# google-ai-edge/ai-edge-quantizer

Measured on AMD Instinct MI355X. Metric: weight-bytes quantized/sec (GB/s), 4096x4096 per-channel int8, higher is better.
Workload: dtype f32; 1 GPU; per-channel int8 symmetric requant of 4096x4096 FP32 weight buffers (BASELINE config 2)

## Files before the change

### ai-edge-quantizer_amd/csrc/reduce_exact.hip

```cpp
#include <cstdlib>

#include "common.h"

namespace mi355q {
namespace {

constexpr int kChunk = 8192;

__device__ __forceinline__ float lane_bcast(float v, int src_lane) {
  return __int_as_float(__builtin_amdgcn_readlane(__float_as_int(v), src_lane));
}

__device__ __forceinline__ float wave_shr1(float v) {
  return __int_as_float(__builtin_amdgcn_update_dpp(0, __float_as_int(v), 0x138, 0xF, 0xF, false));
}

template <bool SQUARE>
__device__ __forceinline__ float tr(float v) {
  if constexpr (SQUARE) return v * v;
  return v;
}

template <bool SQUARE>
__device__ __forceinline__ float leaf_sum(const float* a, int m, int lane) {
  const int full = m & ~7;
  float r = 0.f;
  if (lane < 8) {
    r = tr<SQUARE>(a[lane]);
    for (int i = 8; i < full; i += 8) r = r + tr<SQUARE>(a[i + lane]);
  }
  const float r0 = lane_bcast(r, 0), r1 = lane_bcast(r, 1), r2 = lane_bcast(r, 2),
              r3 = lane_bcast(r, 3), r4 = lane_bcast(r, 4), r5 = lane_bcast(r, 5),
              r6 = lane_bcast(r, 6), r7 = lane_bcast(r, 7);
  float res = ((r0 + r1) + (r2 + r3)) + ((r4 + r5) + (r6 + r7));
  for (int i = full; i < m; ++i) res = res + tr<SQUARE>(a[i]);
  return res;
}

template <bool SQUARE, int DEPTH>
__device__ __noinline__ float pairwise_sum(const float* a, int n, int lane) {
  if (n < 8) {
    float res = 0.f;
    for (int i = 0; i < n; ++i) res = res + tr<SQUARE>(a[i]);
    return res;
  }
  if (n <= 128) return leaf_sum<SQUARE>(a, n, lane);
  if constexpr (DEPTH > 0) {
    int n2 = n / 2;
    n2 -= n2 % 8;
    const float left = pairwise_sum<SQUARE, DEPTH - 1>(a, n2, lane);
    const float right = pairwise_sum<SQUARE, DEPTH - 1>(a + n2, n - n2, lane);
    return left + right;
  } else {
    return leaf_sum<SQUARE>(a, n, lane);
  }
}

struct RunSum {
  float acc = 0.f;
  unsigned count = 0;
  int pend_start = 0;
  int pend_len = 0;
  float pend_sum = 0.f;

  __device__ __forceinline__ void flush(const float* a, int lane) {
    if (pend_len > 0) {
      acc = acc + (pend_len < 8 ? pend_sum : pairwise_sum<false, 8>(a + pend_start, pend_len, lane));
      pend_len = 0;
    }
  }

  __device__ __forceinline__ void feed(unsigned long long m, int base, float v, const float* a,
                                       int lane) {
    if ((base % kChunk) == 0 || (m & 1ull) == 0) flush(a, lane);
    count += static_cast<unsigned>(__builtin_popcountll(m));
    if (m == 0) return;
    const unsigned long long m4 = m & (m >> 1) & (m >> 2) & (m >> 3);
    if ((m4 & (m4 >> 4)) != 0 || (pend_len > 0 && pend_len + __builtin_ctzll(~m) >= 8)) {
      feed_runs(m, base, v, a, lane);
      return;
    }
    const float carry = pend_len > 0 ? pend_sum : 0.f;
    pend_len = 0;
    const bool sel = ((m >> lane) & 1ull) != 0;
    float partial = sel ? (lane == 0 ? carry : 0.f) + v : 0.f;
    const unsigned long long m2 = m & (m >> 1);
    if (m2 != 0) {
      const bool cont = (((m2 << 1) >> lane) & 1ull) != 0;
      const int rounds = (m2 & (m >> 2)) == 0 ? 1 : (m4 == 0 ? 2 : 6);
      for (int t = 0; t < rounds; ++t) {
        const float left = wave_shr1(partial);
        if (cont) partial = left + v;
      }
    }
    unsigned long long mf = m;
    if (m >> 63) {
      const int t = __builtin_clzll(~m);
      mf = m & (~0ull >> t);
      pend_start = base + 64 - t;
      pend_len = t;
      pend_sum = lane_bcast(partial, 63);
    }
    unsigned long long ends = mf & ~(mf >> 1);
    const int k = __builtin_popcountll(ends);
    if (k <= 3) {
      while (ends != 0) {
        acc = acc + lane_bcast(partial, __builtin_ctzll(ends));
        ends &= ends - 1ull;
      }
      return;
    }
    const bool is_end = ((ends >> lane) & 1ull) != 0;
    const int rank = __builtin_amdgcn_mbcnt_hi(static_cast<unsigned>(ends >> 32),
                                               __builtin_amdgcn_mbcnt_lo(static_cast<unsigned>(ends), 0));
    const int dest = is_end ? rank : k + lane - rank;
    const float r = __int_as_float(__builtin_amdgcn_ds_permute(dest << 2, __float_as_int(partial)));
    float x = r;
    for (int t = 0; t < k; t += 4) {
#pragma unroll
      for (int j = 0; j < 4; ++j) {
        const float left = __int_as_float(__builtin_amdgcn_update_dpp(
            __float_as_int(acc), __float_as_int(x), 0x138, 0xF, 0xF, false));
        x = left + r;
      }
    }
    acc = lane_bcast(x, k - 1);
  }

  __device__ __forceinline__ float chain(float start, float v, int s, int len) {
    float rs = start;
    for (int i = 0; i < len; ++i) rs = rs + lane_bcast(v, s + i);
    return rs;
  }

  __device__ __forceinline__ void feed_runs(unsigned long long m, int base, float v, const float* a,
                                            int lane) {
    while (m != 0) {
      const int s = __builtin_ctzll(m);
      const unsigned long long t = m >> s;
      const int len = (~t == 0) ? 64 - s : __builtin_ctzll(~t);
      if (s + len == 64) {
        if (pend_len > 0) {
          pend_len += len;
        } else {
          pend_start = base + s;
          pend_len = len;
          if (len < 8) pend_sum = chain(0.f, v, s, len);
        }
        return;
      }
      if (pend_len > 0) {
        if (pend_len + len < 8) {
          acc = acc + chain(pend_sum, v, 0, len);
          pend_len = 0;
        } else {
          pend_len += len;
          flush(a, lane);
        }
      } else if (len < 8) {
        acc = acc + chain(0.f, v, s, len);
      } else {
        acc = acc + pairwise_sum<false, 8>(a + base + s, len, lane);
      }
      m &= ~(((1ull << len) - 1ull) << s);
    }
  }
};

template <bool USE_LDS>
__device__ __forceinline__ const float* stage_unit(const float* g, int len, float* lds, int lane) {
  if constexpr (!USE_LDS) return g;
  if ((reinterpret_cast<uintptr_t>(g) & 15) == 0) {
    const int n4 = len / 4;
    const float4* g4 = reinterpret_cast<const float4*>(g);
    float4* l4 = reinterpret_cast<float4*>(lds);
    for (int i = lane; i < n4; i += kWave) l4[i] = g4[i];
    for (int i = n4 * 4 + lane; i < len; i += kWave) lds[i] = g[i];
  } else {
    for (int i = lane; i < len; i += kWave) lds[i] = g[i];
  }
  return lds;
}

struct OctavArgs {
  const float* x;
  long long units;
  int len;
  int lds_stride;
  int max_iter;
  int count_is_f64;
  float s;
  float* hist;
  unsigned long long* moving;
  struct TailState* tail;
  float* tail_values;
  unsigned short* tail_pos;
  int tail_cap;
};

struct TailState {
  int next_it;
  int n[2];
  float guess;
  float cand_guess;
  unsigned moved_lo, moved_hi;
  int pad;
};

struct OctavStep {
  float next;
  bool close;
};

__device__ __forceinline__ OctavStep octav_step(float guess, float pos_sum, float neg_sum,
                                                long long pos_count, long long neg_count,
                                                long long len, float s, int count_is_f64) {
  const float num = pos_sum - neg_sum;
  float den = static_cast<float>(pos_count);
  den = static_cast<float>(static_cast<double>(den) + static_cast<double>(neg_count));
  den = den * (1.0f - s);
  if (count_is_f64)
    den = static_cast<float>(static_cast<double>(den) +
                             static_cast<double>(s) * static_cast<double>(len));
  else
    den = den + s * static_cast<float>(len);
  const float next = num / den;
  const float tol = 1e-8f + 1e-5f * fabsf(next);
  const bool close = (fabsf(guess - next) <= tol && __builtin_isfinite(next)) || guess == next;
  return {next, close};
}

__device__ __forceinline__ void publish_moving(unsigned long long* flags, unsigned long long moved) {
  if (moved == 0) return;
  const unsigned long long seen = __atomic_load_n(flags, __ATOMIC_RELAXED);
  if ((seen & moved) != moved) atomicOr(flags, moved);
}

__device__ __forceinline__ bool reached_fixed_point(float guess, float next) { return next == guess; }

__device__ __forceinline__ void repeat_iterate(const OctavArgs& a, int it, long long unit, float value) {
  for (int r = it + 1; r < a.max_iter; ++r) a.hist[static_cast<long long>(r) * a.units + unit] = value;
}

template <bool USE_LDS>
__global__ void octav_kernel(OctavArgs a) {
  extern __shared__ __attribute__((aligned(16))) float smem[];
  const int lane = threadIdx.x & (kWave - 1);
  const int wave = threadIdx.x / kWave;
  const long long unit = static_cast<long long>(blockIdx.x) * (blockDim.x / kWave) + wave;
  const bool live = unit < a.units;
  const float* u = nullptr;
  if (live)
    u = stage_unit<USE_LDS>(a.x + unit * a.len, a.len, smem + static_cast<size_t>(wave) * a.lds_stride, lane);
  if constexpr (USE_LDS) __syncthreads();
  if (!live) return;

  const int len = a.len;
  const float qnan = __builtin_nanf("");
  float guess = 1.0f;
  unsigned long long moved = 0;
  for (int it = 0; it < a.max_iter; ++it) {
    RunSum pos, neg;
    const float hi = guess, lo = -guess;
    for (int base = 0; base < len; base += kWave) {
      const int i = base + lane;
      const float v = i < len ? u[i] : qnan;
      const unsigned long long mp = __ballot(v >= hi), mn = __ballot(v <= lo);
      if ((mp | mn) == 0 && (pos.pend_len | neg.pend_len) == 0) continue;
      pos.feed(mp, base, v, u, lane);
      neg.feed(mn, base, v, u, lane);
    }
    pos.flush(u, lane);
    neg.flush(u, lane);
    const OctavStep st = octav_step(guess, pos.acc, neg.acc, pos.count, neg.count, len, a.s,
                                    a.count_is_f64);
    if (lane == 0) a.hist[static_cast<long long>(it) * a.units + unit] = st.next;
    if (!st.close) moved |= 1ull << it;
    if (reached_fixed_point(guess, st.next)) {
      if (lane == 0) repeat_iterate(a, it, unit, st.next);
      break;
    }
    guess = st.next;
  }
  if (lane == 0) publish_moving(a.moving, moved);
}

#ifndef MI355Q_ROWS_MIN_LEN
#define MI355Q_ROWS_MIN_LEN 129
#endif
constexpr int kRowsMinLen = MI355Q_ROWS_MIN_LEN, kRowsMaxLen = 2 * kChunk;
constexpr int kPiece = 16;

__device__ __forceinline__ int pidx(int e) { return e + (e >> 4); }


template <int CTRL, int ROW_MASK>
__device__ __forceinline__ int dpp_add(int x) {
  return x + __builtin_amdgcn_update_dpp(0, x, CTRL, ROW_MASK, 0xF, true);
}

__device__ __forceinline__ int wave_incl_scan(int x) {
  x = dpp_add<0x111, 0xF>(x);
  x = dpp_add<0x112, 0xF>(x);
  x = dpp_add<0x114, 0xF>(x);
  x = dpp_add<0x118, 0xF>(x);
// ... 1214 lines not shown
}

size_t octav_rows_smem(int len) {
  const int kRowsThreads = octav_rows_threads(len);
  const int npieces = (len + kPiece - 1) / kPiece;
  const size_t row_floats = static_cast<size_t>((len + (len >> 4) + 4) & ~3);
  const size_t cap = static_cast<size_t>(((len / 2 + 2 + 63) & ~63) + 64);
  return 2 * rows_xchg_floats(kRowsThreads) * sizeof(float) + kRowsThreads * sizeof(float) + row_floats * sizeof(float) + cap * 2 * sizeof(float) +
         static_cast<size_t>((npieces + 1) & ~1) * 2 * sizeof(unsigned short);
}

__global__ void octav_seg_kernel(OctavArgs a, long long channels, long long outer) {
  const int lane = threadIdx.x & (kWave - 1);
  const int wave = threadIdx.x / kWave;
  const long long c = static_cast<long long>(blockIdx.x) * (blockDim.x / kWave) + wave;
  if (c >= channels) return;
  const int inner = a.len;
  const float qnan = __builtin_nanf("");
  float guess = 1.0f;
  unsigned long long moved = 0;
  for (int it = 0; it < a.max_iter; ++it) {
    RunSum pos, neg;
    long long npos = 0, nneg = 0;
    const float hi = guess, lo = -guess;
    for (long long o = 0; o < outer; ++o) {
      const float* u = a.x + (o * channels + c) * inner;
      for (int base = 0; base < inner; base += kWave) {
        const int i = base + lane;
        const float v = i < inner ? u[i] : qnan;
        pos.feed(__ballot(v >= hi), base, v, u, lane);
        neg.feed(__ballot(v <= lo), base, v, u, lane);
      }
      pos.flush(u, lane);
      neg.flush(u, lane);
      npos += pos.count;
      nneg += neg.count;
      pos.count = neg.count = 0;
    }
    const OctavStep st = octav_step(guess, pos.acc, neg.acc, npos, nneg, outer * inner, a.s, 1);
    if (lane == 0) a.hist[static_cast<long long>(it) * a.units + c] = st.next;
    if (!st.close) moved |= 1ull << it;
    if (reached_fixed_point(guess, st.next)) {
      if (lane == 0) repeat_iterate(a, it, c, st.next);
      break;
    }
    guess = st.next;
  }
  if (lane == 0) publish_moving(a.moving, moved);
}

__global__ void mse_scale_seg_kernel(const float* __restrict__ x, long long outer, long long channels,
                                     int inner, float multiplier, float* __restrict__ scale) {
  const int lane = threadIdx.x & (kWave - 1);
  const int wave = threadIdx.x / kWave;
  const long long c = static_cast<long long>(blockIdx.x) * (blockDim.x / kWave) + wave;
  if (c >= channels) return;
  float acc = 0.f;
  bool first = true;
  for (long long o = 0; o < outer; ++o) {
    const float* u = x + (o * channels + c) * inner;
    for (int k = 0; k < inner; k += kChunk) {
      const int n = inner - k < kChunk ? inner - k : kChunk;
      const float part = pairwise_sum<true, 8>(u + k, n, lane);
      acc = first ? part : acc + part;
      first = false;
    }
  }
  const float mean = acc / static_cast<float>(outer * inner);
  if (lane == 0) scale[c] = multiplier * __builtin_sqrtf(mean);
}

constexpr int kColsUnroll = 8;

__global__ __launch_bounds__(256) void octav_cols_kernel(OctavArgs a, long long channels) {
  const long long c_raw = static_cast<long long>(blockIdx.x) * 256 + threadIdx.x;
  const bool live = c_raw < channels;
  const long long c = live ? c_raw : channels - 1;
  const long long outer = a.len;
  float guess = 1.0f;
  bool settled = false;
  unsigned long long moved = 0;
  for (int it = 0; it < a.max_iter; ++it) {
    const float hi = guess, lo = -guess;
    float pos = 0.f, neg = 0.f;
    long long npos = 0, nneg = 0;
    const float* p = a.x + c;
    long long o = 0;
    for (; o + kColsUnroll <= outer; o += kColsUnroll) {
      float v[kColsUnroll];
#pragma unroll
      for (int k = 0; k < kColsUnroll; ++k) v[k] = p[static_cast<long long>(k) * channels];
#pragma unroll
      for (int k = 0; k < kColsUnroll; ++k) {
        if (v[k] >= hi) { pos = pos + v[k]; ++npos; }
        if (v[k] <= lo) { neg = neg + v[k]; ++nneg; }
      }
      p += kColsUnroll * channels;
    }
    for (; o < outer; ++o, p += channels) {
      const float v = *p;
      if (v >= hi) { pos = pos + v; ++npos; }
      if (v <= lo) { neg = neg + v; ++nneg; }
    }
    const OctavStep st = octav_step(guess, pos, neg, npos, nneg, outer, a.s, a.count_is_f64);
    if (live && !settled) a.hist[static_cast<long long>(it) * a.units + c] = st.next;
    if (live && !settled && !st.close) moved |= 1ull << it;
    if (!settled && reached_fixed_point(guess, st.next)) {
      settled = true;
      if (live) repeat_iterate(a, it, c, st.next);
    }
    guess = st.next;
    if (__all(settled)) break;
  }
  for (int off = kWave / 2; off > 0; off >>= 1) moved |= __shfl_xor(moved, off, kWave);
  if ((threadIdx.x & (kWave - 1)) == 0) publish_moving(a.moving, moved);
}

__global__ __launch_bounds__(256) void mse_scale_cols_kernel(const float* __restrict__ x, long long outer,
                                                            long long channels, float multiplier,
                                                            float* __restrict__ scale) {
  const long long c = static_cast<long long>(blockIdx.x) * 256 + threadIdx.x;
  if (c >= channels) return;
  const float* p = x + c;
  float acc = 0.f;
  long long o = 0;
  for (; o + kColsUnroll <= outer; o += kColsUnroll) {
    float v[kColsUnroll];
#pragma unroll
    for (int k = 0; k < kColsUnroll; ++k) v[k] = p[static_cast<long long>(k) * channels];
#pragma unroll
    for (int k = 0; k < kColsUnroll; ++k) acc = acc + v[k] * v[k];
    p += kColsUnroll * channels;
  }
  for (; o < outer; ++o, p += channels) acc = acc + (*p) * (*p);
  scale[c] = multiplier * __builtin_sqrtf(acc / static_cast<float>(outer));
}

__global__ __launch_bounds__(256) void octav_pick_kernel(const float* __restrict__ hist,
                                                        const unsigned long long* __restrict__ moving,
                                                        long long units, int max_iter, int early_stop,
                                                        float* __restrict__ clip, int* iters_out) {
  int k = max_iter - 1;
  if (early_stop)
    for (int it = 0; it < max_iter; ++it)
      if (((*moving >> it) & 1ull) == 0) { k = it; break; }
  const long long i = static_cast<long long>(blockIdx.x) * 256 + threadIdx.x;
  if (i < units) clip[i] = hist[static_cast<long long>(k) * units + i];
  if (i == 0 && iters_out != nullptr) *iters_out = k + 1;
}

struct MseArgs {
  const float* x;
  long long units;
  int len;
  int lds_stride;
  float multiplier;
  float* scale;
  unsigned* q = nullptr;
  float lo = 0.f, hi = 0.f;
};

__device__ void list_leaves(int lo, int n, int* leaf_lo, int* leaf_n, int* count) {
  if (n <= 128) {
    leaf_lo[*count] = lo;
    leaf_n[*count] = n;
    ++*count;
    return;
  }
  int n2 = n / 2;
  n2 -= n2 % 8;
  list_leaves(lo, n2, leaf_lo, leaf_n, count);
  list_leaves(lo + n2, n - n2, leaf_lo, leaf_n, count);
}

__device__ float fold_leaves(int n, const float* leaf_sum, int* next) {
  if (n <= 128) return leaf_sum[(*next)++];
  int n2 = n / 2;
  n2 -= n2 % 8;
  const float left = fold_leaves(n2, leaf_sum, next);
  return left + fold_leaves(n - n2, leaf_sum, next);
}

__global__ __launch_bounds__(256) void mse_scale_leaves_kernel(MseArgs a) {
  __shared__ int leaf_lo[2][128], leaf_n[2][128], leaves[2];
  __shared__ float leaf_sum[4][128];
  const int lane = threadIdx.x & (kWave - 1), wave = threadIdx.x / kWave;
  const int k = lane & 7, slot = lane >> 3;
  const int last_len = a.len - (a.len - 1) / kChunk * kChunk;
  if (threadIdx.x == 0 || threadIdx.x == kWave) {
    const int t = threadIdx.x == 0 ? 0 : 1;
    int c = 0;
    list_leaves(0, t == 0 ? (a.len < kChunk ? a.len : kChunk) : last_len, leaf_lo[t], leaf_n[t], &c);
    leaves[t] = c;
  }
  __syncthreads();
  const long long unit = static_cast<long long>(blockIdx.x) * 4 + wave;
  const bool live_unit = unit < a.units;
  const float* u = a.x + (live_unit ? unit : 0) * a.len;
  float acc = 0.f;
  for (int c0 = 0; c0 < a.len; c0 += kChunk) {
    const int n = a.len - c0 < kChunk ? a.len - c0 : kChunk;
    const int t = (c0 + kChunk >= a.len) ? 1 : 0;
    const int count = leaves[t];
    for (int base = 0; base < count; base += 8) {
      const int leaf = base + slot;
      const bool live = leaf < count;
      const float* p = u + c0 + (live ? leaf_lo[t][leaf] : 0);
      const int ln = live ? leaf_n[t][leaf] : 0;
      float res = 0.f;
      if (ln < 8) {
        for (int i = 0; i < ln; ++i) res = res + p[i] * p[i];
      } else {
        float v[16];
#pragma unroll
        for (int q = 0; q < 16; ++q) v[q] = (8 * (q + 1) <= ln) ? p[8 * q + k] : 0.f;
        float r = v[0] * v[0];
#pragma unroll
        for (int q = 1; q < 16; ++q)
          if (8 * (q + 1) <= ln) r = r + v[q] * v[q];
        r = r + __shfl_xor(r, 1, kWave);
        r = r + __shfl_xor(r, 2, kWave);
        r = r + __shfl_xor(r, 4, kWave);
        for (int i = ln & ~7; i < ln; ++i) r = r + p[i] * p[i];
        res = r;
      }
      if (live && k == 0) leaf_sum[wave][leaf] = res;
    }
    __syncthreads();
    if (lane == 0) {
      int next = 0;
      const float part = fold_leaves(n, leaf_sum[wave], &next);
      acc = c0 == 0 ? part : acc + part;
    }
    __syncthreads();
  }
  if (lane == 0 && live_unit) {
    const float mean = acc / static_cast<float>(a.len);
    a.scale[unit] = a.multiplier * __builtin_sqrtf(mean);
  }
}

__global__ __launch_bounds__(256) void mse_scale_balanced_kernel(MseArgs a, int last_leaf, int last_depth) {
  const int lane = threadIdx.x & (kWave - 1), wave = threadIdx.x / kWave;
  const int k = lane & 7, slot = lane >> 3;
  const long long unit = static_cast<long long>(blockIdx.x) * 4 + wave;
  if (unit >= a.units) return;
  const float* u = a.x + unit * a.len;
  float acc = 0.f;
  for (int c0 = 0; c0 < a.len; c0 += kChunk) {
    const bool last = c0 + kChunk >= a.len;
    const int leaf_len = last ? last_leaf : 128, depth = last ? last_depth : 6;
    const int count = 1 << depth;
    const int steps = count > 8 ? count >> 3 : 1;
    float lvl0 = 0.f, lvl1 = 0.f, lvl2 = 0.f, x = 0.f;
#pragma unroll
    for (int s = 0; s < 8; ++s) {
      if (s < steps) {
        const int leaf = s * 8 + slot;
        const float* p = u + c0 + static_cast<long long>(leaf < count ? leaf : 0) * leaf_len + k;
        float v[16];
#pragma unroll
        for (int q = 0; q < 16; ++q) v[q] = (8 * (q + 1) <= leaf_len) ? p[8 * q] : 0.f;
        float r = v[0] * v[0];
#pragma unroll
        for (int q = 1; q < 16; ++q)
          if (8 * (q + 1) <= leaf_len) r = r + v[q] * v[q];
        r = r + __shfl_xor(r, 1, kWave);
        r = r + __shfl_xor(r, 2, kWave);
        r = r + __shfl_xor(r, 4, kWave);
        if (count > 1) r = r + __shfl_xor(r, 8, kWave);
        if (count > 2) r = r + __shfl_xor(r, 16, kWave);
        if (count > 4) r = r + __shfl_xor(r, 32, kWave);
        x = r;
        if (s & 1) {
          x = lvl0 + x;
          if (s & 2) {
            x = lvl1 + x;
            if (s & 4) x = lvl2 + x; else lvl2 = x;
          } else {
            lvl1 = x;
          }
        } else {
          lvl0 = x;
        }
      }
    }
    acc = c0 == 0 ? x : acc + x;
  }
  acc = lane_bcast(acc, 0);
  const float mean = acc / static_cast<float>(a.len);
  const float scale = a.multiplier * __builtin_sqrtf(mean);
  if (lane == 0) a.scale[unit] = scale;
  if (a.q != nullptr) {
    const float4* u4 = reinterpret_cast<const float4*>(u);
    unsigned* q = a.q + unit * (a.len / 4);
    for (int i = lane; i < a.len / 4; i += kWave) {
      const float4 v = u4[i];
      const unsigned w = (static_cast<unsigned>(round_clip(v.x / scale, a.lo, a.hi)) & 0xFFu) |
                         ((static_cast<unsigned>(round_clip(v.y / scale, a.lo, a.hi)) & 0xFFu) << 8) |
                         ((static_cast<unsigned>(round_clip(v.z / scale, a.lo, a.hi)) & 0xFFu) << 16) |
                         ((static_cast<unsigned>(round_clip(v.w / scale, a.lo, a.hi)) & 0xFFu) << 24);
      __builtin_nontemporal_store(w, q + i);
    }
  }
}

struct UnitPlan {
  bool use_lds;
  int waves;
  int lds_stride;
  size_t smem;
};

UnitPlan plan_units(int len) {
  UnitPlan p{};
  const int stride = (len + 3) / 4 * 4;
  const size_t per_wave = static_cast<size_t>(stride) * sizeof(float);
  constexpr size_t kBudget = 64 * 1024;
  int waves = static_cast<int>(kBudget / (per_wave ? per_wave : 1));
  if (waves > 4) waves = 4;
  if (waves >= 1) {
    p.use_lds = true;
    p.waves = waves;
    p.lds_stride = stride;
    p.smem = per_wave * waves;
  } else {
    p.use_lds = false;
    p.waves = 4;
    p.lds_stride = 0;
    p.smem = 0;
  }
  return p;
}


struct OctavFastArgs {
  const float* x;
  long long units;
  int len;
  int max_iter;
  float s;
  float* hist;
  unsigned long long* moving;
};

template <int CTRL>
__device__ __forceinline__ float dpp_f32(float v) {
  return __builtin_bit_cast(float, __builtin_amdgcn_update_dpp(0, __builtin_bit_cast(int, v), CTRL, 0xF, 0xF, true));
}
template <int CTRL>
__device__ __forceinline__ int dpp_i32(int v) { return __builtin_amdgcn_update_dpp(0, v, CTRL, 0xF, 0xF, true); }

template <int LANES>
__device__ __forceinline__ float unit_sum_f32(float v) {
  if constexpr (LANES >= 2) v += dpp_f32<0xB1>(v);
  if constexpr (LANES >= 4) v += dpp_f32<0x4E>(v);
  if constexpr (LANES >= 8) v += dpp_f32<0x141>(v);
  if constexpr (LANES >= 16) v += dpp_f32<0x140>(v);
  if constexpr (LANES >= 32) {
    const int b = __builtin_bit_cast(int, v);
    const float r0 = __builtin_bit_cast(float, __builtin_amdgcn_readlane(b, 0)), r1 = __builtin_bit_cast(float, __builtin_amdgcn_readlane(b, 16));
    const float r2 = __builtin_bit_cast(float, __builtin_amdgcn_readlane(b, 32)), r3 = __builtin_bit_cast(float, __builtin_amdgcn_readlane(b, 48));
    if constexpr (LANES >= 64) v = (r0 + r1) + (r2 + r3);
    else v = (threadIdx.x & 32) ? r2 + r3 : r0 + r1;
  }
  return v;
}
template <int LANES>
__device__ __forceinline__ int unit_sum_i32(int v) {
  if constexpr (LANES >= 2) v += dpp_i32<0xB1>(v);
  if constexpr (LANES >= 4) v += dpp_i32<0x4E>(v);
  if constexpr (LANES >= 8) v += dpp_i32<0x141>(v);
  if constexpr (LANES >= 16) v += dpp_i32<0x140>(v);
  if constexpr (LANES >= 32) {
    const int r0 = __builtin_amdgcn_readlane(v, 0), r1 = __builtin_amdgcn_readlane(v, 16);
    const int r2 = __builtin_amdgcn_readlane(v, 32), r3 = __builtin_amdgcn_readlane(v, 48);
    if constexpr (LANES >= 64) v = (r0 + r1) + (r2 + r3);
    else v = (threadIdx.x & 32) ? r2 + r3 : r0 + r1;
  }
  return v;
}

template <int LANES, int V>
__global__ __launch_bounds__(LANES > 256 ? LANES : 256) void octav_fast_kernel(OctavFastArgs a) {
  constexpr int THREADS = LANES > 256 ? LANES : 256;
  constexpr int UPB = THREADS / LANES;
  constexpr int WAVES = LANES / kWave;
  const int l = threadIdx.x % LANES;
  const long long u = static_cast<long long>(blockIdx.x) * UPB + threadIdx.x / LANES;
  const bool live = u < a.units;
  const int len4 = a.len / 4;
  const float4* __restrict__ x4 = reinterpret_cast<const float4*>(a.x) + (live ? u : 0) * len4;
  const float qnan = __builtin_nanf("");
  typedef float v4f __attribute__((ext_vector_type(4)));
  v4f raw[V];
#pragma unroll
  for (int j = 0; j < V; ++j) {
    const int c = j * LANES + l;
    raw[j] = __builtin_nontemporal_load(reinterpret_cast<const v4f*>(&x4[c < len4 ? c : len4 - 1]));
  }
  float v[V][4];
  int zeros = 0;
  float top = 0.f;
#pragma unroll
  for (int j = 0; j < V; ++j) {
    const bool mine = live && j * LANES + l < len4;
#pragma unroll
    for (int e = 0; e < 4; ++e) {
      v[j][e] = mine ? fabsf(raw[j][e]) : qnan;
      top = fmaxf(top, v[j][e]);
      if constexpr (LANES >= kWave) zeros += __builtin_popcountll(__builtin_amdgcn_ballot_w64(v[j][e] == 0.f));
      else zeros += v[j][e] == 0.f;
    }
  }
  __shared__ double red_sum[2][WAVES > 0 ? WAVES : 1];
  __shared__ int red_cnt[2][WAVES > 0 ? WAVES : 1];
  float unit_top = 0.f;
  if constexpr (LANES >= kWave) {
    unit_top = top;
#pragma unroll
    for (int off = kWave / 2; off > 0; off >>= 1) unit_top = fmaxf(unit_top, __shfl_xor(unit_top, off, kWave));
    if constexpr (WAVES > 1) {
      __shared__ float red_top[WAVES > 0 ? WAVES : 1];
      if ((threadIdx.x & (kWave - 1)) == 0) red_top[threadIdx.x / kWave] = unit_top;
      __syncthreads();
#pragma unroll
      for (int k = 0; k < WAVES; ++k) unit_top = fmaxf(unit_top, red_top[k]);
    }
  }
  float guess = 1.0f;
  unsigned long long moved = 0;
  int it = 0;
  for (; it < a.max_iter; ++it) {
    float part = 0.f;
    int cnt = 0;
    if constexpr (LANES >= kWave) {
      if (!(guess > unit_top)) {
        float p0 = 0.f, p1 = 0.f, p2 = 0.f, p3 = 0.f;
#pragma unroll
        for (int j = 0; j < V; ++j) {
          float t0, t1, t2, t3;
          int n0, n1, n2, n3;
          unsigned long long m0, m1, m2, m3;
          asm volatile(
              "v_cmp_ge_f32_e64 %[m0], %[x0], %[g]\n\tv_cmp_ge_f32_e64 %[m1], %[x1], %[g]\n\t"
              "v_cmp_ge_f32_e64 %[m2], %[x2], %[g]\n\tv_cmp_ge_f32_e64 %[m3], %[x3], %[g]\n\t"
              "v_cndmask_b32_e64 %[t0], 0, %[x0], %[m0]\n\tv_cndmask_b32_e64 %[t1], 0, %[x1], %[m1]\n\t"
              "v_cndmask_b32_e64 %[t2], 0, %[x2], %[m2]\n\tv_cndmask_b32_e64 %[t3], 0, %[x3], %[m3]\n\t"
              "s_bcnt1_i32_b64 %[n0], %[m0]\n\ts_bcnt1_i32_b64 %[n1], %[m1]\n\t"
              "s_bcnt1_i32_b64 %[n2], %[m2]\n\ts_bcnt1_i32_b64 %[n3], %[m3]\n\t"
              "v_add_f32 %[p0], %[p0], %[t0]\n\tv_add_f32 %[p1], %[p1], %[t1]\n\t"
              "v_add_f32 %[p2], %[p2], %[t2]\n\tv_add_f32 %[p3], %[p3], %[t3]\n\t"
              "s_add_i32 %[n0], %[n0], %[n1]\n\ts_add_i32 %[n2], %[n2], %[n3]\n\t"
              "s_add_i32 %[c], %[c], %[n0]\n\ts_add_i32 %[c], %[c], %[n2]"
              : [p0] "+v"(p0), [p1] "+v"(p1), [p2] "+v"(p2), [p3] "+v"(p3), [c] "+s"(cnt),
                [t0] "=&v"(t0), [t1] "=&v"(t1), [t2] "=&v"(t2), [t3] "=&v"(t3),
                [n0] "=&s"(n0), [n1] "=&s"(n1), [n2] "=&s"(n2), [n3] "=&s"(n3),
                [m0] "=&s"(m0), [m1] "=&s"(m1), [m2] "=&s"(m2), [m3] "=&s"(m3)
              : [x0] "v"(v[j][0]), [x1] "v"(v[j][1]), [x2] "v"(v[j][2]), [x3] "v"(v[j][3]), [g] "v"(guess)
              : "scc");
        }
        part = (p0 + p1) + (p2 + p3);
        if (guess == 0.f) cnt += zeros;
      }
    } else {
#pragma unroll
      for (int j = 0; j < V; ++j)
#pragma unroll
        for (int e = 0; e < 4; ++e) {
          const bool sel = v[j][e] >= guess;
          part += sel ? v[j][e] : 0.f;
          cnt += sel;
        }
      cnt = unit_sum_i32<LANES>(cnt + (guess == 0.f ? zeros : 0));
    }
    double sum = static_cast<double>(unit_sum_f32<(LANES < kWave ? LANES : kWave)>(part));
    if constexpr (WAVES > 1) {
      const int w = threadIdx.x / kWave, b = it & 1;
      if ((threadIdx.x & (kWave - 1)) == 0) { red_sum[b][w] = sum; red_cnt[b][w] = cnt; }
      __syncthreads();
      sum = 0.0; cnt = 0;
#pragma unroll
      for (int k = 0; k < WAVES; ++k) { sum += red_sum[b][k]; cnt += red_cnt[b][k]; }
    }
    const OctavStep st = octav_step(guess, static_cast<float>(sum), 0.f, cnt, 0, a.len, a.s, 1);
    if (live && l == 0) a.hist[static_cast<long long>(it) * a.units + u] = st.next;
    if (!st.close) moved |= 1ull << it;
    const bool fixed = reached_fixed_point(guess, st.next);
    guess = st.next;
    if constexpr (LANES >= kWave) {
      if (fixed) { ++it; break; }
    }
  }
  if constexpr (LANES >= kWave) {
    if (live && l == 0)
      for (int k = it; k < a.max_iter; ++k) a.hist[static_cast<long long>(k) * a.units + u] = guess;
  }
  if (!live) moved = 0;
#pragma unroll
  for (int off = kWave / 2; off > 0; off >>= 1) {
    const unsigned lo = __shfl_xor(static_cast<unsigned>(moved), off, kWave);
    const unsigned hi = __shfl_xor(static_cast<unsigned>(moved >> 32), off, kWave);
    moved |= (static_cast<unsigned long long>(hi) << 32) | lo;
  }
  if ((threadIdx.x & (kWave - 1)) == 0) publish_moving(a.moving, moved);
}

template <int LANES, int V>
void launch_octav_fast(const OctavFastArgs& a, hipStream_t st) {
  constexpr int THREADS = LANES > 256 ? LANES : 256;
  constexpr int UPB = THREADS / LANES;
  hipLaunchKernelGGL((octav_fast_kernel<LANES, V>), dim3(static_cast<unsigned>((a.units + UPB - 1) / UPB)), dim3(THREADS), 0, st, a);
}

}
}

using namespace mi355q;

extern "C" size_t mi355q_octav_workspace_bytes(int64_t units, int32_t max_iter) {
  if (units <= 0 || max_iter <= 0) return 0;
  return static_cast<size_t>(units) * max_iter * sizeof(float) + 64 * sizeof(int);
}

extern "C" size_t mi355q_octav_rows_workspace_bytes(int64_t units, int64_t unit_len, int32_t max_iter) {
  const size_t base = mi355q_octav_workspace_bytes(units, max_iter);
  if (base == 0 || unit_len < kRowsMinLen || unit_len > kRowsMaxLen) return base;
  const size_t cap = static_cast<size_t>(octav_tail_cap(static_cast<int>(unit_len)));
  return ((base + 63) & ~static_cast<size_t>(63)) + static_cast<size_t>(units) * (sizeof(TailState) + 2 * cap * (sizeof(float) + sizeof(unsigned short)));
}

extern "C" int32_t mi355q_octav_clip_f32(const float* x, int64_t units, int64_t unit_len,
                                         int32_t bits, int32_t max_iter, float exponent_divisor,
                                         int32_t early_stop, int32_t count_is_f64, float* clip_out,
                                         int32_t* iters_out, void* workspace,
                                         size_t workspace_bytes, void* stream) {
  clear_error();
  if (units < 0 || unit_len < 0) return fail(MI355Q_BAD_ARG, "negative shape");
  if (max_iter < 1 || max_iter > 64) return fail(MI355Q_BAD_ARG, "max_iter must be in [1, 64]");
  if (bits < 1 || bits > 16) return fail(MI355Q_BAD_ARG, "bits must be in [1, 16]");
  if (units == 0) return MI355Q_OK;
  if (unit_len == 0) return fail(MI355Q_BAD_SHAPE, "empty reduction unit");
  if (unit_len > 0x7FFFFFFFLL - 64) return fail(MI355Q_UNSUPPORTED, "unit_len too large");
  if (!x || !clip_out) return fail(MI355Q_BAD_ARG, "null pointer");
  const size_t need = mi355q_octav_workspace_bytes(units, max_iter);
  if (!workspace || workspace_bytes < need)
    return fail(MI355Q_BAD_ARG, "workspace too small: need %zu bytes", need);
  hipStream_t st = as_stream(stream);
  float* hist = static_cast<float*>(workspace);
  unsigned long long* not_close = reinterpret_cast<unsigned long long*>(hist + (units * max_iter + 1) / 2 * 2);
  if (hipMemsetAsync(not_close, 0, sizeof(unsigned long long), st) != hipSuccess)
    return fail(MI355Q_HIP_ERROR, "hipMemsetAsync failed");
  double p4 = 1.0;
  for (int i = 0; i < bits; ++i) p4 *= 0.25;
  const float s = static_cast<float>(p4 / static_cast<double>(exponent_divisor));
  if ((unit_len == 32 || unit_len == 64 || unit_len == 128 || unit_len == 256) && (reinterpret_cast<uintptr_t>(x) & 15) == 0 &&
      (units + kWave - 1) / kWave <= 0x7FFFFFFFLL && octav_unit_lanes_on() && !getenv("MI355Q_OCTAV_WAVE_KERNEL")) {
    OctavArgs a{x, units, static_cast<int>(unit_len), 0, max_iter, count_is_f64, s, hist, not_close};
    const dim3 grid(static_cast<unsigned>((units + kWave - 1) / kWave));
    if (unit_len == 32) hipLaunchKernelGGL(octav_unit_lanes_kernel<32>, grid, dim3(kWave), 0, st, a);
    else if (unit_len == 64) hipLaunchKernelGGL(octav_unit_lanes_kernel<64>, grid, dim3(kWave), 0, st, a);
    else if (unit_len == 128) hipLaunchKernelGGL(octav_unit_lanes_kernel<128>, grid, dim3(kWave), 0, st, a);
    else hipLaunchKernelGGL(octav_unit_lanes_kernel<256>, grid, dim3(kWave), 0, st, a);
    MI355Q_CHECK_LAUNCH("octav unit lanes launch");
    hipLaunchKernelGGL(octav_pick_kernel, dim3(static_cast<unsigned>((units + 255) / 256)), dim3(256), 0, st,
                       hist, not_close, units, max_iter, early_stop, clip_out, iters_out);
    MI355Q_CHECK_LAUNCH("octav pick launch");
    return MI355Q_OK;
  }
  if (unit_len >= kRowsMinLen && unit_len <= kRowsMaxLen && !getenv("MI355Q_OCTAV_WAVE_KERNEL")) {
    static const bool tail_on = [] { const char* e = getenv("MI355Q_OCTAV_TAIL"); return e == nullptr || atoi(e) != 0; }();
    const int threads = octav_rows_threads(static_cast<int>(unit_len));
    OctavArgs a{x, units, static_cast<int>(unit_len), 0, max_iter, count_is_f64, s, hist, not_close, nullptr, nullptr, nullptr, 0};
    a.tail_cap = octav_tail_cap(a.len);
    const int slots_ = ((a.len + kPiece - 1) / kPiece + threads - 1) / threads;
    if (tail_on && slots_ == 1 && workspace_bytes >= mi355q_octav_rows_workspace_bytes(units, unit_len, max_iter)) {
      unsigned char* tb = reinterpret_cast<unsigned char*>(workspace) + ((need + 63) & ~static_cast<size_t>(63));
      a.tail = reinterpret_cast<TailState*>(tb);
      a.tail_values = reinterpret_cast<float*>(tb + static_cast<size_t>(units) * sizeof(TailState));
      a.tail_pos = reinterpret_cast<unsigned short*>(a.tail_values + static_cast<size_t>(units) * 2 * a.tail_cap);
    }
    const size_t smem = octav_rows_smem(a.len);
    const int slots = ((a.len + kPiece - 1) / kPiece + threads - 1) / threads;
    const int variant = threads == 1024 ? 6 : threads == 512 ? 5 : slots;
    const void* fn = variant == 6 ? reinterpret_cast<const void*>(octav_rows_kernel<1, 1024>)
                   : variant == 5 ? reinterpret_cast<const void*>(octav_rows_kernel<1, 512>)
                   : slots == 4 ? reinterpret_cast<const void*>(octav_rows_kernel<4, 256>)
                   : slots == 3 ? reinterpret_cast<const void*>(octav_rows_kernel<3, 256>)
                   : slots == 2 ? reinterpret_cast<const void*>(octav_rows_kernel<2, 256>)
                   : threads == 256 ? reinterpret_cast<const void*>(octav_rows_kernel<1, 256>)
                   : threads == 128 ? reinterpret_cast<const void*>(octav_rows_kernel<1, 128>)
                                    : reinterpret_cast<const void*>(octav_rows_kernel<1, 64>);
    (void)variant;
    if (smem > 64 * 1024) {
      const hipError_t e = hipFuncSetAttribute(fn, hipFuncAttributeMaxDynamicSharedMemorySize, 160 * 1024);
      if (e != hipSuccess) return fail(MI355Q_HIP_ERROR, "hipFuncSetAttribute: %s", hipGetErrorString(e));
    }
    if (units > 0x7FFFFFFFLL) return fail(MI355Q_UNSUPPORTED, "too many units");
    void* kargs[] = {&a};
    if (hipLaunchKernel(fn, dim3(static_cast<unsigned>(units)), dim3(threads), kargs, smem, st) != hipSuccess)
      return fail(MI355Q_HIP_ERROR, "octav rows launch failed");
    MI355Q_CHECK_LAUNCH("octav rows launch");
    if (a.tail != nullptr) {
      hipLaunchKernelGGL(octav_tail_kernel, dim3(static_cast<unsigned>(units)), dim3(kWave), static_cast<size_t>(a.tail_cap) * 12, st, a);
      MI355Q_CHECK_LAUNCH("octav tail launch");
    }
    hipLaunchKernelGGL(octav_pick_kernel, dim3(static_cast<unsigned>((units + 255) / 256)), dim3(256), 0, st,
                       hist, not_close, units, max_iter, early_stop, clip_out, iters_out);
    MI355Q_CHECK_LAUNCH("octav pick launch");
    return MI355Q_OK;
  }
  if (unit_len >= 2 * kPiece && unit_len <= 512 && (unit_len & (unit_len - 1)) == 0 &&
      (units * unit_len) % kGroupLen == 0 && (reinterpret_cast<uintptr_t>(x) & 15) == 0 &&
      units * unit_len / kGroupLen <= 0x7FFFFFFFLL && !getenv("MI355Q_OCTAV_WAVE_KERNEL")) {
    OctavArgs a{x, units, static_cast<int>(unit_len), 0, max_iter, count_is_f64, s, hist, not_close};
    const size_t smem = octav_groups_smem();
    hipLaunchKernelGGL(octav_groups_kernel, dim3(static_cast<unsigned>(units * unit_len / kGroupLen)), dim3(kGroupThreads), smem,
                       st, a, static_cast<int>(unit_len));
    MI355Q_CHECK_LAUNCH("octav groups launch");
    hipLaunchKernelGGL(octav_pick_kernel, dim3(static_cast<unsigned>((units + 255) / 256)), dim3(256), 0, st,
                       hist, not_close, units, max_iter, early_stop, clip_out, iters_out);
    MI355Q_CHECK_LAUNCH("octav pick launch");
    return MI355Q_OK;
  }
  const UnitPlan p = plan_units(static_cast<int>(unit_len));
  OctavArgs a{x, units, static_cast<int>(unit_len), p.lds_stride, max_iter, count_is_f64, s, hist, not_close};
  const dim3 blk(p.waves * kWave);
  const dim3 grid(static_cast<unsigned>((units + p.waves - 1) / p.waves));
  if (p.use_lds)
    hipLaunchKernelGGL(octav_kernel<true>, grid, blk, p.smem, st, a);
  else
    hipLaunchKernelGGL(octav_kernel<false>, grid, blk, 0, st, a);
  MI355Q_CHECK_LAUNCH("octav launch");
  hipLaunchKernelGGL(octav_pick_kernel, dim3(static_cast<unsigned>((units + 255) / 256)), dim3(256), 0, st,
                     hist, not_close, units, max_iter, early_stop, clip_out, iters_out);
  MI355Q_CHECK_LAUNCH("octav pick launch");
  return MI355Q_OK;
}

extern "C" int32_t mi355q_octav_clip_fast_f32(const float* x, int64_t units, int64_t unit_len, int32_t bits,
                                              int32_t max_iter, float exponent_divisor, int32_t early_stop,
                                              float* clip_out, int32_t* iters_out, void* workspace,
                                              size_t workspace_bytes, void* stream) {
  clear_error();
  if (units < 0 || unit_len < 0) return fail(MI355Q_BAD_ARG, "negative shape");
  if (max_iter < 1 || max_iter > 64) return fail(MI355Q_BAD_ARG, "max_iter must be in [1, 64]");
  if (bits < 1 || bits > 16) return fail(MI355Q_BAD_ARG, "bits must be in [1, 16]");
  if (units == 0) return MI355Q_OK;
  if (unit_len == 0) return fail(MI355Q_BAD_SHAPE, "empty reduction unit");
  if (unit_len % 4 != 0 || unit_len > 65536)
    return fail(MI355Q_UNSUPPORTED, "the one-read OCTAV kernel takes units of 4 .. 65536 elements, a multiple of 4 (got %lld):"
                                    " use mi355q_octav_clip_f32", static_cast<long long>(unit_len));
  if (units > 0x7FFFFFFFLL) return fail(MI355Q_UNSUPPORTED, "too many units");
  if (!x || !clip_out) return fail(MI355Q_BAD_ARG, "null pointer");
  if (reinterpret_cast<uintptr_t>(x) & 15u) return fail(MI355Q_BAD_ARG, "x must be 16-byte aligned");
  const size_t need = mi355q_octav_workspace_bytes(units, max_iter);
  if (!workspace || workspace_bytes < need)
    return fail(MI355Q_BAD_ARG, "workspace too small: need %zu bytes", need);
  hipStream_t st = as_stream(stream);
  float* hist = static_cast<float*>(workspace);
  unsigned long long* moving = reinterpret_cast<unsigned long long*>(hist + (units * max_iter + 1) / 2 * 2);
  if (hipMemsetAsync(moving, 0, sizeof(unsigned long long), st) != hipSuccess)
    return fail(MI355Q_HIP_ERROR, "hipMemsetAsync failed");
  double p4 = 1.0;
  for (int i = 0; i < bits; ++i) p4 *= 0.25;
  const float s = static_cast<float>(p4 / static_cast<double>(exponent_divisor));
  const OctavFastArgs a{x, units, static_cast<int>(unit_len), max_iter, s, hist, moving};
  const int len4 = static_cast<int>(unit_len / 4);
  if (len4 <= 4) launch_octav_fast<1, 4>(a, st);
  else if (len4 <= 8) launch_octav_fast<2, 4>(a, st);
  else if (len4 <= 16) launch_octav_fast<4, 4>(a, st);
  else if (len4 <= 32) launch_octav_fast<8, 4>(a, st);
  else if (len4 <= 64) launch_octav_fast<16, 4>(a, st);
  else if (len4 <= 128) launch_octav_fast<32, 4>(a, st);
  else if (len4 <= 256) launch_octav_fast<64, 4>(a, st);
  else if (len4 <= 512) launch_octav_fast<64, 8>(a, st);
  else if (len4 <= 1024) launch_octav_fast<64, 16>(a, st);
  else if (len4 <= 2048) launch_octav_fast<256, 8>(a, st);
  else if (len4 <= 4096) launch_octav_fast<256, 16>(a, st);
  else if (len4 <= 8192) launch_octav_fast<1024, 8>(a, st);
  else launch_octav_fast<1024, 16>(a, st);
  MI355Q_CHECK_LAUNCH("octav one-read launch");
  hipLaunchKernelGGL(octav_pick_kernel, dim3(static_cast<unsigned>((units + 255) / 256)), dim3(256), 0, st,
                     hist, moving, static_cast<long long>(units), max_iter, early_stop, clip_out, iters_out);
  MI355Q_CHECK_LAUNCH("octav pick launch");
  return MI355Q_OK;
}

extern "C" int32_t mi355q_octav_clip_nd_f32(const float* x, int64_t outer, int64_t channels,
                                            int64_t inner, int32_t bits, int32_t max_iter,
                                            float exponent_divisor, int32_t early_stop, float* clip_out,
                                            int32_t* iters_out, void* workspace,
                                            size_t workspace_bytes, void* stream) {
  if (outer == 1)
    return mi355q_octav_clip_f32(x, channels, inner, bits, max_iter, exponent_divisor, early_stop, 1,
                                 clip_out, iters_out, workspace, workspace_bytes, stream);
  clear_error();
  if (outer < 0 || channels < 0 || inner < 0) return fail(MI355Q_BAD_ARG, "negative shape");
  if (max_iter < 1 || max_iter > 64) return fail(MI355Q_BAD_ARG, "max_iter must be in [1, 64]");
  if (bits < 1 || bits > 16) return fail(MI355Q_BAD_ARG, "bits must be in [1, 16]");
  if (channels == 0) return MI355Q_OK;
  if (outer == 0 || inner == 0) return fail(MI355Q_BAD_SHAPE, "empty reduction unit");
  if (outer > 0x7FFFFFFFLL || inner > 0x7FFFFFFFLL - 64 || outer * inner > 0x7FFFFFFFLL)
    return fail(MI355Q_UNSUPPORTED, "reduction unit too large");
  if (!x || !clip_out) return fail(MI355Q_BAD_ARG, "null pointer");
  const size_t need = mi355q_octav_workspace_bytes(channels, max_iter);
  if (!workspace || workspace_bytes < need)
    return fail(MI355Q_BAD_ARG, "workspace too small: need %zu bytes", need);
  hipStream_t st = as_stream(stream);
  float* hist = static_cast<float*>(workspace);
  unsigned long long* not_close = reinterpret_cast<unsigned long long*>(hist + (channels * max_iter + 1) / 2 * 2);
  if (hipMemsetAsync(not_close, 0, sizeof(unsigned long long), st) != hipSuccess)
    return fail(MI355Q_HIP_ERROR, "hipMemsetAsync failed");
  double p4 = 1.0;
  for (int i = 0; i < bits; ++i) p4 *= 0.25;
  const float s = static_cast<float>(p4 / static_cast<double>(exponent_divisor));
  if (inner == 1) {
    OctavArgs a{x, channels, static_cast<int>(outer), 0, max_iter, 1, s, hist, not_close};
    hipLaunchKernelGGL(octav_cols_kernel, dim3(static_cast<unsigned>((channels + 255) / 256)), dim3(256), 0,
                       st, a, static_cast<long long>(channels));
  } else {
    OctavArgs a{x, channels, static_cast<int>(inner), 0, max_iter, 1, s, hist, not_close};
    hipLaunchKernelGGL(octav_seg_kernel, dim3(static_cast<unsigned>((channels + 3) / 4)), dim3(4 * kWave), 0,
                       st, a, static_cast<long long>(channels), static_cast<long long>(outer));
  }
  MI355Q_CHECK_LAUNCH("octav nd launch");
  hipLaunchKernelGGL(octav_pick_kernel, dim3(static_cast<unsigned>((channels + 255) / 256)), dim3(256), 0, st,
                     hist, not_close, static_cast<long long>(channels), max_iter, early_stop, clip_out,
                     iters_out);
  MI355Q_CHECK_LAUNCH("octav pick launch");
  return MI355Q_OK;
}

extern "C" int32_t mi355q_mse_scale_nd_f32(const float* x, int64_t outer, int64_t channels,
                                           int64_t inner, float multiplier, float* scale_out,
                                           void* stream) {
  if (outer == 1) return mi355q_mse_scale_f32(x, channels, inner, multiplier, scale_out, stream);
  clear_error();
  if (outer < 0 || channels < 0 || inner < 0) return fail(MI355Q_BAD_ARG, "negative shape");
  if (channels == 0) return MI355Q_OK;
  if (outer == 0 || inner == 0) return fail(MI355Q_BAD_SHAPE, "empty reduction unit");
  if (inner > 0x7FFFFFFFLL - 64) return fail(MI355Q_UNSUPPORTED, "inner too large");
  if (!x || !scale_out) return fail(MI355Q_BAD_ARG, "null pointer");
  hipStream_t st = as_stream(stream);
  if (inner == 1)
    hipLaunchKernelGGL(mse_scale_cols_kernel, dim3(static_cast<unsigned>((channels + 255) / 256)), dim3(256),
                       0, st, x, static_cast<long long>(outer), static_cast<long long>(channels),
                       multiplier, scale_out);
  else
    hipLaunchKernelGGL(mse_scale_seg_kernel, dim3(static_cast<unsigned>((channels + 3) / 4)), dim3(4 * kWave),
                       0, st, x, static_cast<long long>(outer), static_cast<long long>(channels),
                       static_cast<int>(inner), multiplier, scale_out);
  MI355Q_CHECK_LAUNCH("mse nd launch");
  return MI355Q_OK;
}

extern "C" int32_t mi355q_mse_scale_f32(const float* x, int64_t units, int64_t unit_len,
                                        float multiplier, float* scale_out, void* stream) {
  clear_error();
  if (units < 0 || unit_len < 0) return fail(MI355Q_BAD_ARG, "negative shape");
  if (units == 0) return MI355Q_OK;
  if (unit_len == 0) return fail(MI355Q_BAD_SHAPE, "empty reduction unit");
  if (unit_len > 0x7FFFFFFFLL - 64) return fail(MI355Q_UNSUPPORTED, "unit_len too large");
  if (!x || !scale_out) return fail(MI355Q_BAD_ARG, "null pointer");
  MseArgs a{x, units, static_cast<int>(unit_len), 0, multiplier, scale_out};
  hipStream_t st = as_stream(stream);
  const dim3 grid(static_cast<unsigned>((units + 3) / 4)), blk(4 * kWave);
  int leaf = 0, depth = 0;
  if (balanced_chunk(a.len - (a.len - 1) / kChunk * kChunk, &leaf, &depth))
    hipLaunchKernelGGL(mse_scale_balanced_kernel, grid, blk, 0, st, a, leaf, depth);
  else
    hipLaunchKernelGGL(mse_scale_leaves_kernel, grid, blk, 0, st, a);
  MI355Q_CHECK_LAUNCH("mse_scale launch");
  return MI355Q_OK;
}

extern "C" int32_t mi355q_mse_requant_f32(const float* x, int64_t units, int64_t unit_len, float multiplier, int32_t bits,
                                          int32_t narrow, float* scale_out, int8_t* q_out, void* stream) {
  clear_error();
  if (units < 0 || unit_len < 0) return fail(MI355Q_BAD_ARG, "negative shape");
  if (bits < 2 || bits > 8) return fail(MI355Q_BAD_ARG, "bits must be in [2, 8]");
  if (units == 0) return MI355Q_OK;
  if (unit_len == 0) return fail(MI355Q_BAD_SHAPE, "empty reduction unit");
  if (unit_len > 0x7FFFFFFFLL - 64) return fail(MI355Q_UNSUPPORTED, "unit_len too large");
  if (!x || !scale_out || !q_out) return fail(MI355Q_BAD_ARG, "null pointer");
  int leaf = 0, depth = 0;
  const int len = static_cast<int>(unit_len);
  const bool one_kernel = unit_len % 4 == 0 && (reinterpret_cast<uintptr_t>(x) & 15) == 0 && (reinterpret_cast<uintptr_t>(q_out) & 3) == 0 &&
                          balanced_chunk(len - (len - 1) / kChunk * kChunk, &leaf, &depth) && !getenv("MI355Q_MSE_TWO_KERNELS");
  if (!one_kernel) {
    const int32_t st = mi355q_mse_scale_f32(x, units, unit_len, multiplier, scale_out, stream);
    if (st != MI355Q_OK) return st;
    return mi355q_quantize_f32(x, 1, units, unit_len, scale_out, 0, nullptr, 1, bits, narrow, 8, q_out, stream);
  }
  MseArgs a{x, units, len, 0, multiplier, scale_out};
  a.q = reinterpret_cast<unsigned*>(q_out);
  a.hi = static_cast<float>((1 << (bits - 1)) - 1);
  a.lo = -static_cast<float>(1 << (bits - 1)) + (narrow ? 1.f : 0.f);
  hipLaunchKernelGGL(mse_scale_balanced_kernel, dim3(static_cast<unsigned>((units + 3) / 4)), dim3(4 * kWave), 0, as_stream(stream), a,
                     leaf, depth);
  MI355Q_CHECK_LAUNCH("mse requant launch");
  return MI355Q_OK;
}
```

Baseline: 5101 GB/s.

## Add block-per-row fused MSE scale and int8 requant kernel for common row lengths

Adds a kernel that assigns one 256-thread block to each row. The row is loaded once into registers and squared values are staged through LDS, so the sum-of-squares reduction can run in a fixed tree order across leaves and waves. The same registers are then quantized, and the packed int8 words go out through LDS as 16-byte stores. Previously one wave handled a whole row, which gave little parallelism per row and streamed the row from memory twice; the new path avoids that at the cost of more register pressure and a block-wide sync. It is selected by default for row lengths that are multiples of 1024 up to 16K, and 4096 maps to R=4.

Result: no change. 5097 GB/s (-0.1%).

```diff
diff --git a/ai-edge-quantizer_amd/csrc/reduce_exact.hip b/ai-edge-quantizer_amd/csrc/reduce_exact.hip
--- a/ai-edge-quantizer_amd/csrc/reduce_exact.hip
+++ b/ai-edge-quantizer_amd/csrc/reduce_exact.hip
@@ -1,6 +1,7 @@
 #include <cstdlib>
 
 #include "common.h"
+#include "requant_kernels.h"
 
 namespace mi355q {
 namespace {
@@ -1821,6 +1822,121 @@
                          ((static_cast<unsigned>(round_clip(v.w / scale, a.lo, a.hi)) & 0xFFu) << 24);
       __builtin_nontemporal_store(w, q + i);
     }
+  }
+}
+
+template <int R, int PASS, int L>
+struct MseRowsShape {
+  static_assert(R % PASS == 0 && (PASS * 256) % L == 0 && L % 16 == 0 && L <= 128, "a pass is whole leaves");
+  static constexpr int kPasses = R / PASS;
+  static constexpr int kLeaves = PASS * 256 / L;
+  static constexpr int kChains = kLeaves * 8;
+  static constexpr int kCPL = (kChains + kWave - 1) / kWave;
+  static constexpr int kStride = L + 8;
+  static constexpr int kSlab = kLeaves * kStride;
+  static constexpr int kSubs = kPasses * kCPL;
+  static_assert((kLeaves & (kLeaves - 1)) == 0 && (kSubs & (kSubs - 1)) == 0, "complete trees");
+  static_assert(kChains <= kWave || kChains % kWave == 0, "whole waves of chains");
+  static_assert(kSlab >= kWave * R, "the slab also carries the wave's int8 words");
+};
+
+template <int R, int PASS, int L>
+__global__ __launch_bounds__(256) void mse_requant_rows_kernel(MseArgs a) {
+  using S = MseRowsShape<R, PASS, L>;
+  __shared__ __attribute__((aligned(16))) float slabs[256 / kWave][S::kSlab];
+  __shared__ float part[256 / kWave];
+  const int lane = threadIdx.x & (kWave - 1), wave = threadIdx.x / kWave;
+  const long long row = blockIdx.x;
+  const long long row4 = row * (256 * R);
+  const int run = wave * (kWave * R);
+  const float4* x4 = reinterpret_cast<const float4*>(a.x);
+  float* slab = slabs[wave];
+
+  float4 v[R];
+#pragma unroll
+  for (int j = 0; j < R; ++j) v[j] = requant::gload4<true>(x4 + row4 + run + j * kWave + lane);
+
+  float sub[S::kSubs];
+#pragma unroll
+  for (int p = 0; p < S::kPasses; ++p) {
+#pragma unroll
+    for (int jj = 0; jj < PASS; ++jj) {
+      const float4 t = v[p * PASS + jj];
+      const int e = 4 * (jj * kWave + lane);
+      *reinterpret_cast<float4*>(slab + e + 8 * (e / L)) = make_float4(t.x * t.x, t.y * t.y, t.z * t.z, t.w * t.w);
+    }
+    requant::wave_lds_order();
+#pragma unroll
+    for (int c = 0; c < S::kCPL; ++c) {
+      const int chain = S::kChains < kWave ? (lane & (S::kChains - 1)) : c * kWave + lane;
+      const float* ptr = slab + (chain >> 3) * S::kStride + (chain & 7);
+      float t[L / 8];
+#pragma unroll
+      for (int q = 0; q < L / 8; ++q) t[q] = ptr[8 * q];
+      float r = t[0];
+#pragma unroll
+      for (int q = 1; q < L / 8; ++q) r = r + t[q];
+      r = r + __shfl_xor(r, 1, kWave);
+      r = r + __shfl_xor(r, 2, kWave);
+      r = r + __shfl_xor(r, 4, kWave);
+      if constexpr (S::kLeaves > 1) r = r + __shfl_xor(r, 8, kWave);
+      if constexpr (S::kLeaves > 2) r = r + __shfl_xor(r, 16, kWave);
+      if constexpr (S::kLeaves > 4) r = r + __shfl_xor(r, 32, kWave);
+      sub[p * S::kCPL + c] = r;
+    }
+    requant::wave_lds_order();
+  }
+#pragma unroll
+  for (int s = 1; s < S::kSubs; s *= 2)
+#pragma unroll
+    for (int i = 0; i < S::kSubs; i += 2 * s) sub[i] = sub[i] + sub[i + s];
+  if (lane == 0) part[wave] = sub[0];
+  __syncthreads();
+  const float acc = (part[0] + part[1]) + (part[2] + part[3]);
+  const float mean = acc / static_cast<float>(a.len);
+  const float scale = a.multiplier * __builtin_sqrtf(mean);
+  if (threadIdx.x == 0) *(MI355Q_GLOBAL float*)(a.scale + row) = scale;
+
+  uint32_t w[R];
+#pragma unroll
+  for (int j = 0; j < R; ++j)
+    w[j] = (static_cast<uint32_t>(round_clip(v[j].x / scale, a.lo, a.hi)) & 0xFFu) |
+           ((static_cast<uint32_t>(round_clip(v[j].y / scale, a.lo, a.hi)) & 0xFFu) << 8) |
+           ((static_cast<uint32_t>(round_clip(v[j].z / scale, a.lo, a.hi)) & 0xFFu) << 16) |
+           ((static_cast<uint32_t>(round_clip(v[j].w / scale, a.lo, a.hi)) & 0xFFu) << 24);
+  uint8_t* dst = reinterpret_cast<uint8_t*>(a.q) + (row4 + run) * 4;
+  if (requant::wide_ok(a.q, a.len)) {
+    requant::lds_u32* words = (requant::lds_u32*)slab;
+#pragma unroll
+    for (int j = 0; j < R; ++j) words[j * kWave + lane] = w[j];
+    requant::wave_lds_order();
+    typedef __attribute__((address_space(3))) requant::u32x4_t lds_u32x4;
+#pragma unroll
+    for (int k = 0; k < (R + 3) / 4; ++k) {
+      const int piece = k * kWave + lane;
+      if (R % 4 == 0 || piece < 16 * R) requant::gstore4<false>(dst + piece * 16, *((lds_u32x4*)words + piece));
+    }
+  } else {
+#pragma unroll
+    for (int j = 0; j < R; ++j) requant::store_word<4, true>(dst + (j * kWave + lane) * 4, w[j]);
+  }
+}
+
+bool launch_mse_requant_rows(const MseArgs& a, hipStream_t st) {
+  const dim3 grid(static_cast<unsigned>(a.units)), blk(256);
+  switch (a.len) {
+#define MI355Q_MSE_ROWS(R, PASS, L) \
+    case 1024 * R: hipLaunchKernelGGL((mse_requant_rows_kernel<R, PASS, L>), grid, blk, 0, st, a); return true;
+    MI355Q_MSE_ROWS(2, 2, 128)
+    MI355Q_MSE_ROWS(3, 3, 96)
+    MI355Q_MSE_ROWS(4, 4, 128)
+    MI355Q_MSE_ROWS(5, 5, 80)
+    MI355Q_MSE_ROWS(6, 6, 96)
+    MI355Q_MSE_ROWS(7, 7, 112)
+    MI355Q_MSE_ROWS(8, 4, 128)
+    MI355Q_MSE_ROWS(16, 4, 128)
+#undef MI355Q_MSE_ROWS
+    default: return false;
   }
 }
 
@@ -2316,6 +2432,10 @@
   a.q = reinterpret_cast<unsigned*>(q_out);
   a.hi = static_cast<float>((1 << (bits - 1)) - 1);
   a.lo = -static_cast<float>(1 << (bits - 1)) + (narrow ? 1.f : 0.f);
+  if (!getenv("MI355Q_MSE_WAVE_ROWS") && launch_mse_requant_rows(a, as_stream(stream))) {
+    MI355Q_CHECK_LAUNCH("mse requant rows launch");
+    return MI355Q_OK;
+  }
   hipLaunchKernelGGL(mse_scale_balanced_kernel, dim3(static_cast<unsigned>((units + 3) / 4)), dim3(4 * kWave), 0, as_stream(stream), a,
                      leaf, depth);
   MI355Q_CHECK_LAUNCH("mse requant launch");
```
